# COx2/docker-nvidia-glx-desktop

Hardware: AMD Instinct MI355X
Metric: encoded FPS + p50 end-to-end latency at 1080p60 H.264; concurrent sessions/node (higher is better)
Workload: dtype uint8 video (8-bit 4:2:0), H.264 Constrained Baseline

## Files before the change

### csrc/bindings/module.cpp

```cpp
#include <pybind11/numpy.h>
#include <pybind11/pybind11.h>
#include <pybind11/stl.h>

#include <cstring>

#include "../codec/h264_core.h"
#include "../codec/h264_encoder.h"
#include "../codec/vp8_encoder.h"
#include "../codec/hevc_encoder.h"
#include "../common/hip_check.h"
#include "../common/trace.h"
#include "../kernels/pixel.h"
#include "../runtime/session.h"

namespace py = pybind11;
using namespace mx;

void register_net(py::module& m);
void register_audio(py::module& m);
void register_rfb(py::module& m);

namespace {

template <class T>
T* as_ptr(uintptr_t p) {
    return reinterpret_cast<T*>(p);
}
hipStream_t as_stream(uintptr_t s) { return reinterpret_cast<hipStream_t>(s); }

py::bytes to_bytes(const std::vector<uint8_t>& v) {
    return py::bytes(reinterpret_cast<const char*>(v.data()), v.size());
}

struct PyBits {
    std::vector<uint32_t> words;
    h264::BitWriter w;
    PyBits() : words(4096) { w.init(words.data()); }
    py::tuple finish() {
        const uint32_t bits = w.bits;
        w.flush();
        std::vector<uint8_t> out;
        for (uint32_t i = 0; i < (bits + 7) / 8; ++i) out.push_back((uint8_t)(words[i / 4] >> (24 - 8 * (i % 4))));
        return py::make_tuple(to_bytes(out), bits);
    }
};

py::tuple cavlc_block_py(const std::vector<int>& coef, int nc) {
    PyBits b;
    int16_t c[16] = {0};
    const int n = (int)coef.size();
    if (n != 4 && n != 15 && n != 16) throw std::invalid_argument("block must have 4, 15 or 16 coefficients");
    for (int i = 0; i < n; ++i) c[i] = (int16_t)coef[i];
    h264::cavlc_block(b.w, c, n, nc);
    return b.finish();
}

py::array_t<int> fdct_py(py::array_t<int, py::array::c_style | py::array::forcecast> x) {
    if (x.size() != 16) throw std::invalid_argument("need 16 values");
    py::array_t<int> y(16);
    h264::fdct4x4(x.data(), y.mutable_data());
    return y;
}
py::array_t<int> idct_py(py::array_t<int, py::array::c_style | py::array::forcecast> x) {
    if (x.size() != 16) throw std::invalid_argument("need 16 values");
    py::array_t<int> y(16);
    h264::idct4x4(x.data(), y.mutable_data());
    return y;
}

py::array_t<uint8_t> copy_plane(const uint8_t* dev, int pitch, int w, int h) {
    py::array_t<uint8_t> out({h, w});
    HIP_CHECK(hipDeviceSynchronize());
    HIP_CHECK(hipMemcpy2D(out.mutable_data(), w, dev, pitch, w, h, hipMemcpyDeviceToHost));
    return out;
}

}

PYBIND11_MODULE(_native, m) {
    m.doc() = "mxdesk native runtime: HIP kernels (gfx950), H.264 encoder, session pipeline";

    m.def("device_count", []() {
        int n = 0;
        if (hipGetDeviceCount(&n) != hipSuccess) return 0;
        return n;
    });
    m.def("set_device", [](int d) { HIP_CHECK(hipSetDevice(d)); });
    m.def("device_name", [](int d) {
        hipDeviceProp_t p;
        HIP_CHECK(hipGetDeviceProperties(&p, d));
        return std::string(p.gcnArchName) + " / " + p.name;
    });
    m.def("synchronize", []() { HIP_CHECK(hipDeviceSynchronize()); });
    register_net(m);
    register_audio(m);
    register_rfb(m);
    m.def("now_us", &Session::now_us, "CLOCK_MONOTONIC microseconds (same clock as time.monotonic())");

    py::module h = m.def_submodule("h264", "H.264 building blocks (for tests)");
    h.def("hpel_planes", [](py::array_t<uint8_t, py::array::c_style> ref, int coded_w) {
        if (ref.ndim() != 2 || coded_w % 16 || ref.shape(0) % 16 || ref.shape(1) < coded_w)
            throw std::invalid_argument("ref must be (coded_h, pitch) with 16-aligned coded size");
        int hp = 0;
        auto planes = h264::hpel_planes_for_test(ref.data(), coded_w, (int)ref.shape(0), (int)ref.shape(1), &hp);
        const int rows = (int)ref.shape(0) + 2 * h264::kHpelPad;
        py::list out;
        for (auto& p : planes) {
            py::array_t<uint8_t> a({rows, hp});
            std::memcpy(a.mutable_data(), p.data(), p.size());
            out.append(a);
        }
        return out;
    });
    h.def("mc_luma_gpu", [](py::array_t<uint8_t, py::array::c_style> ref, int coded_w, int x4, int y4) {
        if (ref.ndim() != 2 || coded_w % 16 || ref.shape(0) % 16 || ref.shape(1) < coded_w)
            throw std::invalid_argument("ref must be (coded_h, pitch) with 16-aligned coded size");
        py::array_t<uint8_t> out({16, 16});
        h264::mc_luma_for_test(ref.data(), coded_w, (int)ref.shape(0), (int)ref.shape(1), x4, y4, out.mutable_data());
        return out;
    }, py::arg("ref"), py::arg("coded_w"), py::arg("x4"), py::arg("y4"),
          "16x16 luma prediction at quarter-sample position (x4, y4) by k_inter_encode's interpolation");
    h.def("cavlc_block", &cavlc_block_py, py::arg("coef"), py::arg("nc"));
    h.def("fdct4x4", &fdct_py);
    h.def("idct4x4", &idct_py);
    h.def("ue", [](uint32_t k) {
        PyBits b;
        h264::put_ue(b.w, k);
        return b.finish();
    });
    h.def("se", [](int v) {
        PyBits b;
        h264::put_se(b.w, v);
        return b.finish();
    });
    h.def("luma_qpel", [](py::array_t<uint8_t, py::array::c_style> plane, int x4, int y4) {
        if (plane.ndim() != 2) throw std::invalid_argument("2-D plane");
        const int H = (int)plane.shape(0), W = (int)plane.shape(1);
        return h264::luma_qpel(plane.data(), W, W, H, x4, y4);
    });
    h.def("level_for", &h264::pick_level);
    h.def("zero_sum_4x4", [](int qp) { return h264::zero_sum_4x4(qp); }, py::arg("qp"));
    h.def("zero_sum_chroma_dc", [](int qpc) { return h264::zero_sum_chroma_dc(qpc); }, py::arg("qpc"));
    h.def("chroma_qp", [](int qp, int offset) { return h264::chroma_qp(qp, offset); }, py::arg("qp"),
          py::arg("offset") = 0);
    h.def("quant4x4", [](py::array_t<int, py::array::c_style | py::array::forcecast> y, int qp, bool intra, int start) {
        if (y.size() != 16) throw std::invalid_argument("need 16 values");
        py::array_t<int> z(16);
        const int nz = h264::quant4x4(y.data(), z.mutable_data(), qp, intra, start);
        return py::make_tuple(z, nz);
    }, py::arg("y"), py::arg("qp"), py::arg("intra") = false, py::arg("start") = 0);
    h.def("quant_dc_chroma", [](py::array_t<int, py::array::c_style | py::array::forcecast> dc, int qpc, bool intra) {
        if (dc.size() != 4) throw std::invalid_argument("need 4 values");
        py::array_t<int> z(4);
        const int nz = h264::quant_dc_chroma(dc.data(), z.mutable_data(), qpc, intra);
        return py::make_tuple(z, nz);
    }, py::arg("dc"), py::arg("qpc"), py::arg("intra") = false);
    h.def("luma_block_inter", [](py::array_t<int, py::array::c_style | py::array::forcecast> res, int qp) {
        if (res.size() != 16) throw std::invalid_argument("need 16 values");
        py::array_t<int> z(16), rr(16);
        const int nz = h264::luma_block_inter(res.data(), qp, z.mutable_data(), rr.mutable_data());
        return py::make_tuple(z, rr, nz);
    }, py::arg("res"), py::arg("qp"), "inter luma block: residual (raster) -> levels (scan), reconstructed residual, nz");

    py::class_<h264::EncoderConfig>(m, "EncoderConfig")
        .def(py::init<>())
        .def_readwrite("width", &h264::EncoderConfig::width)
        .def_readwrite("height", &h264::EncoderConfig::height)
        .def_readwrite("fps", &h264::EncoderConfig::fps)
        .def_readwrite("bitrate_kbps", &h264::EncoderConfig::bitrate_kbps)
        .def_readwrite("qp", &h264::EncoderConfig::qp)
        .def_readwrite("qp_min", &h264::EncoderConfig::qp_min)
        .def_readwrite("qp_max", &h264::EncoderConfig::qp_max)
        .def_readwrite("keyint", &h264::EncoderConfig::keyint)
        .def_readwrite("search_range", &h264::EncoderConfig::search_range)
        .def_readwrite("scroll_range", &h264::EncoderConfig::scroll_range)
        .def_readwrite("me_coarse", &h264::EncoderConfig::me_coarse)
        .def_readwrite("intra4x4", &h264::EncoderConfig::intra4x4)
        .def_readwrite("subpel", &h264::EncoderConfig::subpel)
        .def_readwrite("chroma_qp_offset", &h264::EncoderConfig::chroma_qp_offset)
        .def_readwrite("pipeline_depth", &h264::EncoderConfig::pipeline_depth)
        .def_readwrite("aq", &h264::EncoderConfig::aq)
        .def_readwrite("intra_in_p", &h264::EncoderConfig::intra_in_p)
        .def_readwrite("vp8_bpred", &h264::EncoderConfig::vp8_bpred)
        .def_readwrite("vp8_intra", &h264::EncoderConfig::vp8_intra)
        .def_readwrite("mask_x0", &h264::EncoderConfig::mask_x0)
        .def_readwrite("mask_y0", &h264::EncoderConfig::mask_y0)
        .def_readwrite("mask_x1", &h264::EncoderConfig::mask_x1)
        .def_readwrite("mask_y1", &h264::EncoderConfig::mask_y1)
        .def_readwrite("deblock", &h264::EncoderConfig::deblock)
        .def_readwrite("partitions", &h264::EncoderConfig::partitions)
        .def_readwrite("tu_split", &h264::EncoderConfig::tu_split)
        .def_readwrite("hevc_slice_cost", &h264::EncoderConfig::hevc_slice_cost)
        .def_readwrite("hevc_wpp", &h264::EncoderConfig::hevc_wpp)
        .def_readwrite("hevc_wpp_rows", &h264::EncoderConfig::hevc_wpp_rows)
        .def_readwrite("sao", &h264::EncoderConfig::sao)
        .def_readwrite("hevc_chroma_keep", &h264::EncoderConfig::hevc_chroma_keep)
        .def_readwrite("hevc_intra_split", &h264::EncoderConfig::hevc_intra_split);

    py::class_<h264::FrameStats>(m, "FrameStats")
        .def_readonly("frame_index", &h264::FrameStats::frame_index)
        .def_readonly("idr", &h264::FrameStats::idr)
        .def_readonly("qp", &h264::FrameStats::qp)
        .def_readonly("bytes", &h264::FrameStats::bytes)
        .def_readonly("skipped_mbs", &h264::FrameStats::skipped_mbs)
        .def_readonly("encode_ms", &h264::FrameStats::encode_ms)
        .def_property_readonly("sse", [](const h264::FrameStats& s) { return py::make_tuple(s.sse[0], s.sse[1], s.sse[2]); })
        .def_readonly("sse_masked", &h264::FrameStats::sse_masked)
        .def_readonly("masked_pixels", &h264::FrameStats::masked_pixels)
        .def_readonly("deblocked", &h264::FrameStats::deblocked)
        .def_readonly("db_coherent", &h264::FrameStats::db_coherent)
        .def_readonly("db_changed", &h264::FrameStats::db_changed)
        .def_readonly("db_moving", &h264::FrameStats::db_moving)
        .def_readonly("scroll_dx", &h264::FrameStats::scroll_dx)
        .def_readonly("scroll_dy", &h264::FrameStats::scroll_dy);

    py::class_<h264::CpuH264Encoder>(m, "CpuH264Encoder")
        .def(py::init<const h264::EncoderConfig&>())
        .def(
            "encode",
            [](h264::CpuH264Encoder& e, py::array_t<uint8_t, py::array::c_style> y,
               py::array_t<uint8_t, py::array::c_style> uv, bool force_idr) {
                if (y.ndim() != 2 || uv.ndim() != 2 || y.shape(1) != uv.shape(1))
                    throw std::invalid_argument("y (H,P) and uv (H/2,P) planes with equal pitch");
// ... 697 lines not shown
```

### csrc/codec/h264_core.h

```cpp
#pragma once
#include <hip/hip_runtime.h>
#include <stdint.h>

#include "h264_tables.h"

#define MXHD __host__ __device__ __forceinline__

namespace mx {
namespace h264 {

struct BitWriter {
    uint32_t* words;
    uint32_t nwords;
    uint64_t acc;
    int nacc;
    uint32_t bits;

    MXHD void init(uint32_t* w) {
        words = w;
        nwords = 0;
        acc = 0;
        nacc = 0;
        bits = 0;
    }
// ... 455 lines not shown
MXHD Mv predict_mv_skip(MvNb a, MvNb b, MvNb c) {
    if (!a.avail || !b.avail) return Mv{0, 0};
    if (a.ref == 0 && a.mv.x == 0 && a.mv.y == 0) return Mv{0, 0};
    if (b.ref == 0 && b.mv.x == 0 && b.mv.y == 0) return Mv{0, 0};
    return predict_mv16x16(a, b, c);
}

MXHD int cbp_to_codenum(int cbp, bool intra) {
    const uint8_t* t = intra ? kCodeNumToCbpIntra : kCodeNumToCbpInter;
    for (int i = 0; i < 48; ++i)
        if (t[i] == cbp) return i;
    return 0;
}

MXHD int clip255(int v) { return v < 0 ? 0 : (v > 255 ? 255 : v); }

MXHD int ref_px(const uint8_t* p, int pitch, int w, int h, int x, int y) {
    x = x < 0 ? 0 : (x >= w ? w - 1 : x);
    y = y < 0 ? 0 : (y >= h ? h - 1 : y);
    return p[y * pitch + x];
}

MXHD int tap6(int a, int b, int c, int d, int e, int f) { return a - 5 * b + 20 * c + 20 * d - 5 * e + f; }

MXHD int half_h1(const uint8_t* p, int pitch, int w, int h, int x, int y) {
    return tap6(ref_px(p, pitch, w, h, x - 2, y), ref_px(p, pitch, w, h, x - 1, y), ref_px(p, pitch, w, h, x, y),
                ref_px(p, pitch, w, h, x + 1, y), ref_px(p, pitch, w, h, x + 2, y), ref_px(p, pitch, w, h, x + 3, y));
}
MXHD int half_v1(const uint8_t* p, int pitch, int w, int h, int x, int y) {
    return tap6(ref_px(p, pitch, w, h, x, y - 2), ref_px(p, pitch, w, h, x, y - 1), ref_px(p, pitch, w, h, x, y),
                ref_px(p, pitch, w, h, x, y + 1), ref_px(p, pitch, w, h, x, y + 2), ref_px(p, pitch, w, h, x, y + 3));
}

MXHD int luma_qpel(const uint8_t* p, int pitch, int w, int h, int x4, int y4) {
    const int xi = x4 >> 2, yi = y4 >> 2, xf = x4 & 3, yf = y4 & 3;
    const int G = ref_px(p, pitch, w, h, xi, yi);
    if ((xf | yf) == 0) return G;
    auto b_at = [&](int yy) { return clip255((half_h1(p, pitch, w, h, xi, yy) + 16) >> 5); };
    auto h_at = [&](int xx) { return clip255((half_v1(p, pitch, w, h, xx, yi) + 16) >> 5); };
    auto j_val = [&]() {
        int j1 = tap6(half_h1(p, pitch, w, h, xi, yi - 2), half_h1(p, pitch, w, h, xi, yi - 1),
                      half_h1(p, pitch, w, h, xi, yi), half_h1(p, pitch, w, h, xi, yi + 1),
                      half_h1(p, pitch, w, h, xi, yi + 2), half_h1(p, pitch, w, h, xi, yi + 3));
        return clip255((j1 + 512) >> 10);
    };
    if (yf == 0) {
        const int b = b_at(yi);
        if (xf == 2) return b;
        const int other = (xf == 1) ? G : ref_px(p, pitch, w, h, xi + 1, yi);
        return (other + b + 1) >> 1;
    }
    if (xf == 0) {
        const int hh = h_at(xi);
        if (yf == 2) return hh;
        const int other = (yf == 1) ? G : ref_px(p, pitch, w, h, xi, yi + 1);
        return (other + hh + 1) >> 1;
    }
    if (xf == 2 && yf == 2) return j_val();
    if (xf == 2) {
        const int bb = (yf == 1) ? b_at(yi) : b_at(yi + 1);
        return (bb + j_val() + 1) >> 1;
    }
    if (yf == 2) {
        const int hh = (xf == 1) ? h_at(xi) : h_at(xi + 1);
        return (hh + j_val() + 1) >> 1;
    }
    const int bb = (yf == 1) ? b_at(yi) : b_at(yi + 1);
    const int hh = (xf == 1) ? h_at(xi) : h_at(xi + 1);
    return (bb + hh + 1) >> 1;
}

MXHD int chroma_pred8(const uint8_t* uv, int pitch, int cw, int ch, int comp, int x8, int y8) {
    const int xi = x8 >> 3, yi = y8 >> 3, xf = x8 & 7, yf = y8 & 7;
    auto g = [&](int x, int y) {
        x = x < 0 ? 0 : (x >= cw ? cw - 1 : x);
        y = y < 0 ? 0 : (y >= ch ? ch - 1 : y);
        return (int)uv[y * pitch + 2 * x + comp];
    };
    if ((xf | yf) == 0) return g(xi, yi);
    const int A = g(xi, yi), B = g(xi + 1, yi), C = g(xi, yi + 1), D = g(xi + 1, yi + 1);
    return ((8 - xf) * (8 - yf) * A + xf * (8 - yf) * B + (8 - xf) * yf * C + xf * yf * D + 32) >> 6;
}

MXHD int lambda_sad(int qp) {
    constexpr uint8_t tab[52] = {1,  1,  1,  1,  1,  1,  1,  1,  1,  1,  1,  1,  1,  1,  1,  1,  1,  1,
                                 2,  2,  2,  2,  3,  3,  3,  4,  4,  4,  5,  6,  6,  7,  8,  9,  10, 11,
                                 13, 14, 16, 18, 20, 23, 25, 29, 32, 36, 40, 45, 51, 57, 64, 72};
    return tab[qp < 0 ? 0 : (qp > 51 ? 51 : qp)];
}

MXHD int mvd_bits(int d) { return se_len(d); }

}
}
```

### csrc/codec/h264_kernels.hip

```cpp
#include <hip/hip_runtime.h>

#include <cstddef>

#include "../common/hip_check.h"
#include "../common/wave.h"
#include "h264_core.h"
#include "h264_deblock.h"
#include "h264_gpu.h"
#include "h264_mb.h"

namespace mx {
namespace h264 {

namespace {

__device__ __forceinline__ uint32_t bswap32(uint32_t v) { return __builtin_bswap32(v); }

constexpr int kHpTW = 128, kHpTH = 16;
constexpr int kHpSW = kHpTW + 8;
__device__ __forceinline__ int byte_of(uint32_t w, int k) { return (int)((w >> (8 * k)) & 0xff); }
__device__ __forceinline__ uint32_t pack4(int a, int b, int c, int d) {
    const uint32_t lo = __builtin_amdgcn_perm((uint32_t)b, (uint32_t)a, 0x0c0c0400u);
    const uint32_t hi = __builtin_amdgcn_perm((uint32_t)d, (uint32_t)c, 0x0c0c0400u);
    return __builtin_amdgcn_perm(hi, lo, 0x05040100u);
// ... 102 lines not shown
__device__ __forceinline__ int qpel_lds(const uint8_t (*sp)[18][kSpW], int x4, int y4) {
    const int xi = x4 >> 2, yi = y4 >> 2, xf = x4 & 3, yf = y4 & 3;
    const int G = sp[0][yi][xi];
    if ((xf | yf) == 0) return G;
    if (yf == 0) {
        const int b = sp[1][yi][xi];
        if (xf == 2) return b;
        return ((xf == 1 ? G : (int)sp[0][yi][xi + 1]) + b + 1) >> 1;
    }
    if (xf == 0) {
        const int hh = sp[2][yi][xi];
        if (yf == 2) return hh;
        return ((yf == 1 ? G : (int)sp[0][yi + 1][xi]) + hh + 1) >> 1;
    }
    if (xf == 2 && yf == 2) return sp[3][yi][xi];
    if (xf == 2) return ((yf == 1 ? (int)sp[1][yi][xi] : (int)sp[1][yi + 1][xi]) + sp[3][yi][xi] + 1) >> 1;
    if (yf == 2) return ((xf == 1 ? (int)sp[2][yi][xi] : (int)sp[2][yi][xi + 1]) + sp[3][yi][xi] + 1) >> 1;
    const int bb = (yf == 1) ? sp[1][yi][xi] : sp[1][yi + 1][xi];
    const int hh = (xf == 1) ? sp[2][yi][xi] : sp[2][yi][xi + 1];
    return (bb + hh + 1) >> 1;
}

constexpr int kMaxRange = 32;
constexpr int kWinPadX = 4, kWinPadY = 3;
constexpr int kWinStride = 16 + 2 * kMaxRange + 8;
constexpr int kWinRows = 16 + 2 * kMaxRange + 7;
constexpr int kWinWords = kWinRows * kWinStride / 4;

constexpr int kMeThreads = 256, kMeWaves = kMeThreads / 64;
__device__ __forceinline__ uint64_t qsad4(uint32_t hi, uint32_t lo, uint32_t src, uint64_t acc) {
    return __builtin_amdgcn_qsad_pk_u16_u8(((uint64_t)hi << 32) | lo, src, acc);
}
constexpr int kFpRows = 18 + 5;
__device__ __forceinline__ void build_footprints(const uint8_t* win, int org0, int org1, int n,
                                                 uint8_t (*sp)[4][18][kSpW], int16_t (*b1)[kFpRows][kSpW], int tid) {
    for (int i = tid; i < n * kFpRows * 18; i += kMeThreads) {
        const int pi = i / (kFpRows * 18), rem = i - pi * (kFpRows * 18), r = rem / 18, c = rem - r * 18;
        const uint8_t* p = win + (pi ? org1 : org0) + (r - 2) * kWinStride + c;
        b1[pi][r][c] = (int16_t)tap6(p[-2], p[-1], p[0], p[1], p[2], p[3]);
    }
    __syncthreads();
    for (int i = tid; i < n * 324; i += kMeThreads) {
        const int pi = i / 324, rem = i - pi * 324, r = rem / 18, c = rem - r * 18;
        const uint8_t* p = win + (pi ? org1 : org0) + r * kWinStride + c;
        const int16_t(*b)[kSpW] = b1[pi];
        const int v1 = tap6(p[-2 * kWinStride], p[-kWinStride], p[0], p[kWinStride], p[2 * kWinStride], p[3 * kWinStride]);
        const int j1 = tap6(b[r][c], b[r + 1][c], b[r + 2][c], b[r + 3][c], b[r + 4][c], b[r + 5][c]);
        sp[pi][0][r][c] = p[0];
        sp[pi][1][r][c] = (uint8_t)clip255((b[r + 2][c] + 16) >> 5);
        sp[pi][2][r][c] = (uint8_t)clip255((v1 + 16) >> 5);
        sp[pi][3][r][c] = (uint8_t)clip255((j1 + 512) >> 10);
    }
}

struct MeState {
    const uint8_t* ref;
    int qp, search_range, subpel, me_coarse, partitions;
};
__device__ __forceinline__ MeState me_state(const FrameState& f) {
    return MeState{f.me_ref ? f.me_ref : f.ref_y, f.qp, f.search_range, f.subpel, f.me_coarse, f.partitions};
}
__device__ __forceinline__ uint32_t zero_sad_wave(const uint8_t* __restrict__ src_y, const uint8_t* __restrict__ ref,
                                                  int pitch, int x0, int y0, int tid, uint32_t* sw) {
    const int r = tid >> 2, c4 = (tid & 3) * 4;
    *sw = *reinterpret_cast<const uint32_t*>(src_y + (y0 + r) * pitch + x0 + c4);
    const uint32_t rw = *reinterpret_cast<const uint32_t*>(ref + (y0 + r) * pitch + x0 + c4);
    return (uint32_t)wave_sum((int)__builtin_amdgcn_sad_u8(*sw, rw, 0u));
}
__device__ __forceinline__ unsigned long long kmin(unsigned long long a, unsigned long long c) { return c < a ? c : a; }
__device__ __forceinline__ unsigned long long block_min(const unsigned long long* slot) {
    unsigned long long b = slot[0];
    for (int i = 1; i < kMeWaves; ++i) b = kmin(b, slot[i]);
    return b;
}
__device__ __forceinline__ void me_row(const uint32_t* win32, const uint32_t* srcw, int a, int r, uint64_t& lft,
                                       uint64_t& rgt) {
    const uint32_t w0 = win32[a], w1 = win32[a + 1], w2 = win32[a + 2], w3 = win32[a + 3], w4 = win32[a + 4];
    const uint32_t s0 = srcw[r * 4 + 0], s1 = srcw[r * 4 + 1], s2 = srcw[r * 4 + 2], s3 = srcw[r * 4 + 3];
    lft = qsad4(w1, w0, s0, lft);
    lft = qsad4(w2, w1, s1, lft);
    rgt = qsad4(w3, w2, s2, rgt);
    rgt = qsad4(w4, w3, s3, rgt);
}
template <bool kCoarse, class Visit>
__device__ __forceinline__ void me_score16(const uint32_t* win32, const uint32_t* srcw, int ntask, int gw, int side,
                                           int tid, Visit visit) {
    constexpr int kStep = kCoarse ? 2 : 1, kUnroll = kCoarse ? 4 : 2;
    for (int q = tid; q < ntask; q += kMeThreads) {
        const int dyr = kStep * (q / gw), g = q % gw;
        uint64_t acc = 0;
#pragma unroll kUnroll
        for (int r = 0; r < 16; ++r) me_row(win32, srcw, (dyr + r) * (kWinStride / 4) + g, r, acc, acc);
#pragma unroll
        for (int sh = 0; sh < 4; sh += kStep) {
            const int dxr = 4 * g + sh;
            if (dxr >= side) break;
            visit((uint32_t)(acc >> (16 * sh)) & 0xffffu, dxr, dyr);
        }
    }
}
template <int kLanes, class Sad, class Key>
__device__ __forceinline__ unsigned long long me_neighbour(unsigned long long centre, int k, int side, Sad sad,
                                                           Key mkey) {
    const int cb0 = (int)(centre & 0xffff), bxr = cb0 % side, byr = cb0 / side;
    int ddx, ddy;
    subpel_offset(k, &ddx, &ddy);
    const int nxr = bxr + ddx, nyr = byr + ddy;
    const bool inside = nxr >= 0 && nxr < side && nyr >= 0 && nyr < side;
    int d = inside ? sad(nxr, nyr) : 0;
    for (int o = kLanes / 2; o > 0; o >>= 1) d += __shfl_xor(d, o, 64);
    return inside ? mkey((uint32_t)d, nxr, nyr) : ~0ull;
}
template <int kN>
__device__ __forceinline__ void me_refine(const uint8_t (*sp)[4][18][kSpW], uint32_t (*cand)[8], const uint32_t* srcw,
                                          int pi, int k, int sub, int xx, int yy, int lambda, int* vx, int* vy,
                                          uint32_t* cost, bool on = true) {
    const uint32_t s0 = srcw[yy * 4 + (xx >> 2)], s1 = srcw[yy * 4 + (xx >> 2) + 1];
    const int base_x4 = xx * 4 + 4 - vx[pi], base_y4 = yy * 4 + 4 - vy[pi];
    for (int step = 2; step >= 1; step >>= 1) {
        int ddx, ddy;
        subpel_offset(k, &ddx, &ddy);
        const int cx = vx[pi] + ddx * step, cy = vy[pi] + ddy * step;
        int d = 0;
#pragma unroll
        for (int j = 0; j < 8; ++j) {
            d += abs(byte_of(j < 4 ? s0 : s1, j & 3) - qpel_lds(sp[pi], base_x4 + 4 * j + cx, base_y4 + cy));
        }
        if (!on) d = 0;
        for (int o = kMeThreads / (16 * kN); o > 0; o >>= 1) d += __shfl_xor(d, o, 64);
        __syncthreads();
        if (sub == 0) cand[pi][k] = me_cost((uint32_t)d, lambda, cx, cy);
        __syncthreads();
        for (int q = 0; q < kN; ++q) {
            int bdx = 0, bdy = 0;
            uint32_t bcost = cost[q];
            for (int kk = 0; kk < 8; ++kk) {
                const uint32_t cc = cand[q][kk];
                if (cc < bcost) {
                    int ex, ey;
                    subpel_offset(kk, &ex, &ey);
                    bcost = cc;
                    bdx = ex * step;
                    bdy = ey * step;
                }
            }
            vx[q] += bdx;
            vy[q] += bdy;
            cost[q] = bcost;
        }
    }
}
__device__ __forceinline__ MbInfo store_motion(MbInfo* __restrict__ mbs, int mbi, int tid, int cx, int cy, int mvx,
                                               int mvy, int part, const int (&pvx)[2], const int (&pvy)[2]) {
    MbInfo out;
    out.mvx = (int16_t)(4 * cx + mvx);
    out.mvy = (int16_t)(4 * cy + mvy);
    out.part = (uint8_t)part;
    for (int i = 0; i < 2; ++i) {
        out.pmv[2 * i] = part == kPart16x16 ? 0 : (int16_t)(4 * cx + pvx[i]);
        out.pmv[2 * i + 1] = part == kPart16x16 ? 0 : (int16_t)(4 * cy + pvy[i]);
    }
    if (tid == 0) {
        MbInfo& m = mbs[mbi];
        m.mvx = out.mvx;
        m.mvy = out.mvy;
        m.part = out.part;
        for (int i = 0; i < 4; ++i) m.pmv[i] = out.pmv[i];
    }
    return out;
}
__device__ __forceinline__ MbInfo store_motion(MbInfo* __restrict__ mbs, int mbi, int tid, int cx, int cy, int mvx,
                                               int mvy) {
    const int none[2] = {0, 0};
    return store_motion(mbs, mbi, tid, cx, cy, mvx, mvy, kPart16x16, none, none);
}
__device__ __forceinline__ MbInfo store_motion_quads(MbInfo* __restrict__ mbs, int mbi, int tid, int cx, int cy,
                                                     const int (&qvx)[4], const int (&qvy)[4]) {
    MbInfo out;
    out.part = kPart8x8;
#pragma unroll
    for (int q = 0; q < 4; ++q) set_quad_mv(out, q, 4 * cx + qvx[q], 4 * cy + qvy[q]);
    if (tid == 0) {
// ... 25 lines not shown
    const int R = me_range(st.search_range);
    const int W = 16 + 2 * R;
    const uint8_t* __restrict__ ref = st.ref;
    const int lambda = lambda_sad(st.qp);

    constexpr int kWs4 = kWinStride / 4;
    int cx = 0, cy = 0;
    {
        if (tid < 64) {
            uint32_t sw;
            const uint32_t d = zero_sad_wave(src_y, ref, g.pitch, x0, y0, tid, &sw);
            if (tid == 0) s_sad0[0] = d;
        }
        __syncthreads();
        const uint32_t sad0 = s_sad0[0];
        if (sad0 <= static_sad(st.qp)) {
            MbInfo out;
            out.mvx = out.mvy = 0;
            out.part = kPart16x16;
            out.pmv[0] = out.pmv[1] = out.pmv[2] = out.pmv[3] = 0;
            if (tid == 0) {
                MbInfo& m = mbs[mbi];
                m.mvx = 0;
                m.mvy = 0;
                m.part = kPart16x16;
                m.pmv[0] = m.pmv[1] = m.pmv[2] = m.pmv[3] = 0;
            }
            return out;
        }
        if constexpr (kScroll) {
            const int gx = hint[0], gy = hint[1];
            if (gx | gy) {
                if (tid < 64) {
                    const int r = tid >> 2, c4 = (tid & 3) * 4;
                    const uint32_t sw = *reinterpret_cast<const uint32_t*>(src_y + (y0 + r) * g.pitch + x0 + c4);
                    uint32_t rw = 0;
                    for (int k = 0; k < 4; ++k)
                        rw |= (uint32_t)ref_px(ref, g.pitch, g.coded_w, g.coded_h, x0 + gx + c4 + k, y0 + gy + r) << (8 * k);
                    const int d = wave_sum((int)__builtin_amdgcn_sad_u8(sw, rw, 0u));
                    if (tid == 0) s_sad0[1] = (uint32_t)d;
                }
                __syncthreads();
                const int use = scroll_use(s_sad0[1], sad0, st.qp);
                if (use == kScrollExit) return store_motion(mbs, mbi, tid, gx, gy, 0, 0);
                if (use == kScrollCentre) cx = gx, cy = gy;
            }
        }
    }
    const int wrows = W + 2 * kWinPadY + 1, wx0 = x0 + cx - R - kWinPadX, wy0 = y0 + cy - R - kWinPadY;
    const bool dwords = (g.pitch & 3) == 0 && (reinterpret_cast<uintptr_t>(ref) & 3) == 0;
    for (int i = tid; i < wrows * kWs4; i += kMeThreads) {
        const int wy = i / kWs4, wx4 = (i - wy * kWs4) * 4;
        uint32_t w = 0u;
        if (wx4 < W + 2 * kWinPadX) {
            const int py = min(max(wy0 + wy, 0), g.coded_h - 1), px = wx0 + wx4;
            const uint8_t* row = ref + (size_t)py * g.pitch;
            if (kScroll && (wx0 & 3))
                for (int k = 0; k < 4; ++k) w |= (uint32_t)row[min(max(px + k, 0), g.coded_w - 1)] << (8 * k);
            else if (px < 0)
                w = row[0] * 0x01010101u;
            else if (px >= g.coded_w)
                w = row[g.coded_w - 1] * 0x01010101u;
            else if (dwords)
                w = *reinterpret_cast<const uint32_t*>(row + px);
            else
                w = row[px] | ((uint32_t)row[px + 1] << 8) | ((uint32_t)row[px + 2] << 16) | ((uint32_t)row[px + 3] << 24);
        }
        win_lds[i] = w;
    }
    const uint32_t* win32 = win_lds + kWinPadY * kWs4 + kWinPadX / 4;
    auto fp_org = [&](int vx, int vy) {
        return ((vy >> 2) + R + kWinPadY - 1) * kWinStride + (vx >> 2) + R + kWinPadX - 1;
    };
    if (tid < 64) {
        const int r = tid >> 2, c = (tid & 3) * 4;
        srcw[tid] = *reinterpret_cast<const uint32_t*>(src_y + (y0 + r) * g.pitch + x0 + c);
    }
    __syncthreads();

    const int side = 2 * R + 1, gw = (side + 3) >> 2, ngroups = side * gw;
    unsigned long long best = ~0ull;
    const bool coarse = st.me_coarse != 0;
    const bool parts = st.partitions != 0;
    auto mkey = [&](uint32_t sad, int dxr, int dyr) {
        const int dx = dxr - R, dy = dyr - R;
        const uint32_t cost = me_cost(sad, lambda, 4 * dx, 4 * dy);
        const uint32_t dist = (uint32_t)(abs(dx) + abs(dy));
        return ((unsigned long long)cost << 32) | (dist << 16) | (uint32_t)(dyr * side + dxr);
    };
    unsigned long long pb[4] = {~0ull, ~0ull, ~0ull, ~0ull};
    unsigned long long qb[4] = {~0ull, ~0ull, ~0ull, ~0ull};
    auto visit_quads = [&](const uint32_t* qd, int dxr, int dyr) {
        if constexpr (kQuad)
            for (int i = 0; i < 4; ++i) qb[i] = kmin(qb[i], mkey(qd[i], dxr, dyr));
        best = kmin(best, mkey(qd[0] + qd[1] + qd[2] + qd[3], dxr, dyr));
        pb[0] = kmin(pb[0], mkey(qd[0] + qd[1], dxr, dyr));
        pb[1] = kmin(pb[1], mkey(qd[2] + qd[3], dxr, dyr));
        pb[2] = kmin(pb[2], mkey(qd[0] + qd[2], dxr, dyr));
        pb[3] = kmin(pb[3], mkey(qd[1] + qd[3], dxr, dyr));
    };
    if (parts) {
        const int nsh = coarse ? 2 : 4, ntp = coarse ? (R + 1) * gw : ngroups;
        for (int q = tid; q < ntp; q += kMeThreads) {
            const int dyr = coarse ? 2 * (q / gw) : q / gw, g = q % gw;
            uint64_t acc[4] = {0, 0, 0, 0};
#pragma unroll
            for (int h = 0; h < 2; ++h)
#pragma unroll 2
                for (int r = 8 * h; r < 8 * h + 8; ++r)
                    me_row(win32, srcw, (dyr + r) * kWs4 + g, r, acc[2 * h], acc[2 * h + 1]);
#pragma unroll
            for (int si = 0; si < 4; ++si) {
                if (si >= nsh) break;
                const int dxr = 4 * g + (coarse ? 2 * si : si);
                if (dxr >= side) break;
                const int sh = 16 * (coarse ? 2 * si : si);
                const uint32_t qd[4] = {(uint32_t)(acc[0] >> sh) & 0xffffu, (uint32_t)(acc[1] >> sh) & 0xffffu,
                                        (uint32_t)(acc[2] >> sh) & 0xffffu, (uint32_t)(acc[3] >> sh) & 0xffffu};
                visit_quads(qd, dxr, dyr);
            }
        }
    } else {
        auto visit = [&](uint32_t sad, int dxr, int dyr) { best = kmin(best, mkey(sad, dxr, dyr)); };
        if (coarse)
            me_score16<true>(win32, srcw, (R + 1) * gw, gw, side, tid, visit);
        else
            me_score16<false>(win32, srcw, ngroups, gw, side, tid, visit);
    }
    best = wave_min_u64(best);
    if (lane == 0) red[tid >> 6] = best;
    __shared__ unsigned long long pred4[4][kMeWaves];
    if (parts) {
#pragma unroll
        for (int sh = 0; sh < 4; ++sh) {
            const unsigned long long v = wave_min_u64(pb[sh]);
            if (lane == 0) pred4[sh][tid >> 6] = v;
        }
    }
    __shared__ unsigned long long qred4[kQuad ? 4 : 1][kMeWaves];
    if constexpr (kQuad) {
        if (parts) {
#pragma unroll
            for (int i = 0; i < 4; ++i) {
                const unsigned long long v = wave_min_u64(qb[i]);
                if (lane == 0) qred4[i][tid >> 6] = v;
            }
        }
    }
    __syncthreads();
    unsigned long long b = block_min(red);
    unsigned long long pbest[4] = {~0ull, ~0ull, ~0ull, ~0ull};
    if (parts)
        for (int sh = 0; sh < 4; ++sh) pbest[sh] = block_min(pred4[sh]);
    unsigned long long qbest[4] = {~0ull, ~0ull, ~0ull, ~0ull};
    if constexpr (kQuad) {
        if (parts)
            for (int i = 0; i < 4; ++i) qbest[i] = block_min(qred4[i]);
    }
    const uint8_t* wb = reinterpret_cast<const uint8_t*>(win32);
    const uint8_t* sb = reinterpret_cast<const uint8_t*>(srcw);
    if (parts && coarse) {
        __shared__ unsigned long long pnkey[4][8];
        const int ev = tid >> 3, sub = tid & 7, sh = ev >> 3, k = ev & 7;
        const unsigned long long nk = me_neighbour<8>(pbest[sh], k, side, [&](int nxr, int nyr) {
            int d = 0;
            for (int part_row = 0; part_row < 2; ++part_row) {
                const int rr = sh < 2 ? (sh == 0 ? sub : 8 + sub) : 2 * sub + part_row;
                const int c0 = sh < 2 ? 8 * part_row : (sh == 2 ? 0 : 8);
#pragma unroll
                for (int j = 0; j < 8; ++j)
                    d += abs((int)sb[rr * 16 + c0 + j] - (int)wb[(nyr + rr) * kWinStride + nxr + c0 + j]);
            }
            return d;
        }, mkey);
        if (sub == 0) pnkey[sh][k] = nk;
        __syncthreads();
        for (int s2 = 0; s2 < 4; ++s2)
            for (int i = 0; i < 8; ++i) pbest[s2] = kmin(pbest[s2], pnkey[s2][i]);
        if constexpr (kQuad) {
            __shared__ unsigned long long qnkey[4][8];
            const int qi = ev >> 3;
            const unsigned long long qk = me_neighbour<8>(qbest[qi], k, side, [&](int nxr, int nyr) {
                const int rr = 8 * (qi >> 1) + sub, c0 = 8 * (qi & 1);
                int d = 0;
#pragma unroll
                for (int j = 0; j < 8; ++j)
                    d += abs((int)sb[rr * 16 + c0 + j] - (int)wb[(nyr + rr) * kWinStride + nxr + c0 + j]);
                return d;
            }, mkey);
            if (sub == 0) qnkey[qi][k] = qk;
            __syncthreads();
            for (int s2 = 0; s2 < 4; ++s2)
                for (int i = 0; i < 8; ++i) qbest[s2] = kmin(qbest[s2], qnkey[s2][i]);
        }
    }
    if (coarse) {
        __shared__ unsigned long long nkey[8];
        const int k = tid >> 5, sub = tid & 31, py = sub >> 1, px0 = (sub & 1) * 8;
        const unsigned long long nk = me_neighbour<32>(b, k, side, [&](int nxr, int nyr) {
            const uint8_t* wrow = wb + (nyr + py) * kWinStride + nxr + px0;
            const uint32_t s0 = srcw[py * 4 + (px0 >> 2)], s1 = srcw[py * 4 + (px0 >> 2) + 1];
            int d = 0;
#pragma unroll
            for (int j = 0; j < 8; ++j) d += abs(byte_of(j < 4 ? s0 : s1, j & 3) - (int)wrow[j]);
            return d;
        }, mkey);
        if (sub == 0) nkey[k] = nk;
        __syncthreads();
        for (int i = 0; i < 8; ++i) b = kmin(b, nkey[i]);
    }
// ... 2307 lines not shown
```

### csrc/codec/h264_mb.h

```cpp
#pragma once
#include "h264_core.h"
#include "h264_gpu.h"
#include "h264_intra.h"

namespace mx {
namespace h264 {

constexpr int kNumRoles = 28;

struct Avail {
    bool left, top, topright, topleft;
};

MXHD Avail mb_avail(const Geometry& g, int mbx, int mby, int slice_rows) {
    Avail a;
    const bool top_same_slice = mby > 0 && (mby / slice_rows) == ((mby - 1) / slice_rows);
    a.left = mbx > 0;
    a.top = top_same_slice;
    a.topright = top_same_slice && mbx < g.mb_w - 1;
    a.topleft = top_same_slice && mbx > 0;
    return a;
}

MXHD int combine_nc(bool ha, int na, bool hb, int nb) {
// ... 312 lines not shown
            const Mv v = quad_mv(m, q);
            bits += mvd_bits(v.x) + mvd_bits(v.y);
        }
        return satd + (uint32_t)(lambda_sad(frame_qp) * bits);
    }
    return satd + (uint32_t)(lambda_sad(frame_qp) *
                             (mvd_bits(m.pmv[0]) + mvd_bits(m.pmv[1]) + mvd_bits(m.pmv[2]) + mvd_bits(m.pmv[3])));
}

MXHD int idr_slice_rows(int mb_h) {
    const int ns = (mb_h + 3) / 4;
    return (mb_h + ns - 1) / ns;
}

MXHD int qp_delta(int qp, int pred) { return ((qp - pred + 26 + 52) % 52) - 26; }

MXHD SliceParams make_slice_params(int first_mb, int idr, int frame_num, int log2_max_frame_num, int idr_pic_id,
                                   int qp_delta, int deblock_off) {
    SliceParams sp;
    sp.first_mb = first_mb;
    sp.idr = idr;
    sp.frame_num = frame_num;
    sp.log2_max_frame_num = log2_max_frame_num;
    sp.idr_pic_id = idr_pic_id;
    sp.qp_delta = qp_delta;
    sp.disable_deblock = deblock_off;
    return sp;
}


MXHD int luma_block_inter(const int* res, int qp, int* zscan, int* rres) {
    int y[16], z[16], d[16];
    fdct4x4(res, y);
    const int nz = quant4x4(y, z, qp, false, 0);
    for (int k = 0; k < 16; ++k) zscan[k] = z[kZigzag4x4[k]];
    dequant4x4(z, d, qp, 0);
    idct4x4(d, rres);
    return nz;
}

constexpr int fdct_row_gain(int i) { return (i & 1) ? 2 : 1; }
constexpr int zero_sum_4x4_calc(int qp) {
    const int qm = qp % 6, qbits = 15 + qp / 6;
    const int room = (1 << qbits) - 1 - (1 << qbits) / 6;
    int t = room;
    for (int i = 0; i < 16; ++i) {
        const int b = room / (fdct_row_gain(i >> 2) * fdct_row_gain(i & 3) * kQuantMF[qm][kPosClass[i]]);
        t = b < t ? b : t;
    }
    return t;
}
constexpr int zero_sum_chroma_dc_calc(int qpc) {
    const int qm = qpc % 6, qbits = 16 + qpc / 6;
    const int room = (1 << qbits) - 1 - 2 * ((1 << (qbits - 1)) / 6);
    return room / kQuantMF[qm][0];
}
struct ZeroSumTab {
    uint16_t blk[52], cdc[52];
    constexpr ZeroSumTab() : blk{}, cdc{} {
        for (int q = 0; q < 52; ++q) {
            const int a = zero_sum_4x4_calc(q), b = zero_sum_chroma_dc_calc(q);
            blk[q] = (uint16_t)(a > 0xffff ? 0xffff : a);
            cdc[q] = (uint16_t)(b > 0xffff ? 0xffff : b);
        }
    }
};
MXHD int zero_sum_4x4(int qp) {
    constexpr ZeroSumTab tab;
    return tab.blk[qp < 0 ? 0 : (qp > 51 ? 51 : qp)];
}
MXHD int zero_sum_chroma_dc(int qpc) {
    constexpr ZeroSumTab tab;
    return tab.cdc[qpc < 0 ? 0 : (qpc > 51 ? 51 : qpc)];
}

MXHD uint32_t me_cost(uint32_t sad, int lambda, int mvx, int mvy) {
    return sad + (uint32_t)(lambda * (mvd_bits(mvx) + mvd_bits(mvy)));
}

MXHD int me_range(int r) {
    r = r < 4 ? 4 : (r > 32 ? 32 : r);
    return (r + 3) & ~3;
}
constexpr uint32_t kStaticSad = 128;
MXHD uint32_t static_sad(int qp) {
    const uint32_t t = 64u * (uint32_t)lambda_sad(qp);
    return t > kStaticSad ? t : kStaticSad;
}

constexpr int kScrollMaxReach = 192;
MXHD int scroll_reach(int r) {
    r = r < 0 ? 0 : (r > kScrollMaxReach ? kScrollMaxReach : r);
    return (r + 3) & ~3;
}
constexpr int kScrollLattice = 2;
MXHD bool scroll_is_probe(int mbx, int mby) { return mbx % kScrollLattice == 0 && mby % kScrollLattice == 0; }
MXHD int scroll_probes_x(int mb_w) { return (mb_w + kScrollLattice - 1) / kScrollLattice; }
MXHD int scroll_probes_y(int mb_h) { return (mb_h + kScrollLattice - 1) / kScrollLattice; }
constexpr uint32_t kScrollMinVotes = 3;
MXHD int scroll_bins(int D) { return 2 * (2 * D + 1); }
MXHD int scroll_bin(int axis, int d, int D) { return axis * (2 * D + 1) + d + D; }
MXHD unsigned long long scroll_probe_key(uint32_t sad, int axis, int d, int D) {
    const uint32_t ad = (uint32_t)(d < 0 ? -d : d);
    return ((unsigned long long)sad << 32) | (ad << 16) | (uint32_t)scroll_bin(axis, d, D);
}
MXHD bool scroll_key_votes(unsigned long long k, int qp) { return (uint32_t)(k >> 32) <= static_sad(qp); }
MXHD int scroll_key_bin(unsigned long long k) { return (int)(k & 0xffffu); }
MXHD unsigned long long scroll_bin_key(uint32_t votes, int bin, int D) {
    if (!votes) return 0ull;
    const int axis = bin / (2 * D + 1), d = bin % (2 * D + 1) - D;
    const uint32_t ad = (uint32_t)(d < 0 ? -d : d);
    return ((unsigned long long)votes << 32) | ((0xfffu - ad) << 16) | ((uint32_t)(1 - axis) << 15) |
           ((uint32_t)(d < 0) << 14) | (uint32_t)bin;
}
MXHD void scroll_decide(unsigned long long best, uint32_t total, int D, int* gx, int* gy) {
    const uint32_t votes = (uint32_t)(best >> 32);
    *gx = *gy = 0;
    if (votes < kScrollMinVotes || 2u * votes < total) return;
    const int bin = (int)(best & 0x3fffu), axis = bin / (2 * D + 1), d = bin % (2 * D + 1) - D;
    if (axis) *gx = d; else *gy = d;
}
static_assert(2 * (2 * kScrollMaxReach + 1) < (1 << 14), "scroll_bin_key keeps the bin in 14 bits");
enum ScrollUse : int { kScrollExit = 0, kScrollCentre = 1, kScrollZero = 2 };
MXHD int scroll_use(uint32_t sadg, uint32_t sad0, int qp) {
    return sadg <= static_sad(qp) ? kScrollExit : (sadg < sad0 ? kScrollCentre : kScrollZero);
}

MXHD void subpel_offset(int k, int* dx, int* dy) {
    *dx = (k < 3) ? (k - 1) : (k == 3 ? -1 : (k == 4 ? 1 : (k - 6)));
    *dy = (k < 3) ? -1 : ((k == 3 || k == 4) ? 0 : 1);
}

}
}
```

Before: 13250.

## Pack motion-search candidate keys into 32 bits and widen once per thread

The full-search motion estimation kernel now compares candidates with a 32-bit key: cost, distance, and a small per-thread visit number packed together. The MV-bit cost per axis is precomputed with a clz formula, and the winner is decoded back to the 64-bit key only once per thread before the wave reduction. This replaces 64-bit key building and compares (cost, abs, multiply) in the hot inner loop with cheap 32-bit adds and mins, including for partition and quad minima. Static asserts bound the field widths and Python bindings check ordering equivalence, but correctness depends on the packing matching the task map exactly.

```diff
diff --git a/csrc/bindings/module.cpp b/csrc/bindings/module.cpp
--- a/csrc/bindings/module.cpp
+++ b/csrc/bindings/module.cpp
@@ -44,6 +44,46 @@
         return py::make_tuple(to_bytes(out), bits);
     }
 };
+
+py::tuple me_key_check_py(int R, int lambda, bool coarse, const std::vector<uint32_t>& sads) {
+    using namespace h264;
+    if (R != me_range(R)) throw std::invalid_argument("R must be a search range me_range() returns");
+    const int side = 2 * R + 1, gw = me_group_width(R), ntask = me_tasks(R, coarse), step = coarse ? 2 : 1;
+    const uint32_t nmask = (1u << kMeKeyNumBits) - 1;
+    long long bad = 0, pairs = 0;
+    int most = 0;
+    struct Cand { uint32_t term; int dxr, dyr; };
+    for (int tid = 0; tid < kMeSearchThreads; ++tid) {
+        std::vector<Cand> v;
+        uint32_t n0 = 0;
+        for (int q = tid; q < ntask; q += kMeSearchThreads, n0 += 4) {
+            const int dyr = step * (q / gw), g = q % gw;
+            const uint32_t ty = me_key_axis(lambda, dyr - R) + n0;
+            for (int sh = 0; sh < 4; sh += step) {
+                const int dxr = 4 * g + sh;
+                if (dxr >= side) break;
+                v.push_back({ty + me_key_axis(lambda, dxr - R) + (uint32_t)sh, dxr, dyr});
+            }
+        }
+        most = std::max(most, (int)v.size());
+        if (v.empty() && me_key_widen(~0u, tid, R, coarse) != ~0ull) ++bad;
+        for (size_t i = 0; i < v.size(); ++i) {
+            if (i && v[i].dyr * side + v[i].dxr <= v[i - 1].dyr * side + v[i - 1].dxr) ++bad;
+            if (i && (v[i].term & nmask) <= (v[i - 1].term & nmask)) ++bad;
+            for (size_t j = i; j < v.size(); ++j)
+                for (uint32_t sa : sads)
+                    for (uint32_t sb : sads) {
+                        const uint32_t na = me_key32(sa, v[i].term), nb = me_key32(sb, v[j].term);
+                        const unsigned long long wa = me_key64(sa, lambda, R, v[i].dxr, v[i].dyr),
+                                                 wb = me_key64(sb, lambda, R, v[j].dxr, v[j].dyr);
+                        ++pairs;
+                        if ((na < nb) != (wa < wb) || (na == nb) != (wa == wb)) ++bad;
+                        if (me_key_widen(std::min(na, nb), tid, R, coarse) != std::min(wa, wb)) ++bad;
+                    }
+        }
+    }
+    return py::make_tuple(bad, pairs, most);
+}
 
 py::tuple cavlc_block_py(const std::vector<int>& coef, int nc) {
     PyBits b;
@@ -139,6 +179,24 @@
         return h264::luma_qpel(plane.data(), W, W, H, x4, y4);
     });
     h.def("level_for", &h264::pick_level);
+    h.def("me_range", [](int r) { return h264::me_range(r); });
+    h.def("lambda_sad", [](int qp) { return h264::lambda_sad(qp); });
+    h.def("mvd_bits", [](int d) { return h264::mvd_bits(d); });
+    h.def("me_mvd_bits4", [](int d) { return h264::me_mvd_bits4(d); });
+    h.def("me_tasks", [](int R, bool coarse) { return h264::me_tasks(R, coarse); }, py::arg("R"), py::arg("coarse"));
+    h.def("me_key64", [](uint32_t sad, int lambda, int R, int dxr, int dyr) {
+        return h264::me_key64(sad, lambda, R, dxr, dyr);
+    }, py::arg("sad"), py::arg("lambda_"), py::arg("R"), py::arg("dxr"), py::arg("dyr"));
+    h.def("me_key_axis", [](int lambda, int d) { return h264::me_key_axis(lambda, d); });
+    h.def("me_key32", [](uint32_t sad, uint32_t term) { return h264::me_key32(sad, term); });
+    h.def("me_key_widen", [](uint32_t key, int tid, int R, bool coarse) {
+        return h264::me_key_widen(key, tid, R, coarse);
+    }, py::arg("key"), py::arg("tid"), py::arg("R"), py::arg("coarse"));
+    h.def("me_key_check", &me_key_check_py, py::arg("R"), py::arg("lambda_"), py::arg("coarse"), py::arg("sads"));
+    h.attr("ME_MAX_RANGE") = h264::kMeMaxRange;
+    h.attr("ME_SEARCH_THREADS") = h264::kMeSearchThreads;
+    h.attr("ME_MAX_LAMBDA") = h264::kMeMaxLambda;
+    h.attr("ME_KEY_BITS") = py::make_tuple(h264::kMeKeyNumBits, h264::kMeKeyDistBits, h264::kMeKeyCostBits);
     h.def("zero_sum_4x4", [](int qp) { return h264::zero_sum_4x4(qp); }, py::arg("qp"));
     h.def("zero_sum_chroma_dc", [](int qpc) { return h264::zero_sum_chroma_dc(qpc); }, py::arg("qpc"));
     h.def("chroma_qp", [](int qp, int offset) { return h264::chroma_qp(qp, offset); }, py::arg("qp"),
diff --git a/csrc/codec/h264_core.h b/csrc/codec/h264_core.h
--- a/csrc/codec/h264_core.h
+++ b/csrc/codec/h264_core.h
@@ -561,7 +561,7 @@
     return ((8 - xf) * (8 - yf) * A + xf * (8 - yf) * B + (8 - xf) * yf * C + xf * yf * D + 32) >> 6;
 }
 
-MXHD int lambda_sad(int qp) {
+MXHD constexpr int lambda_sad(int qp) {
     constexpr uint8_t tab[52] = {1,  1,  1,  1,  1,  1,  1,  1,  1,  1,  1,  1,  1,  1,  1,  1,  1,  1,
                                  2,  2,  2,  2,  3,  3,  3,  4,  4,  4,  5,  6,  6,  7,  8,  9,  10, 11,
                                  13, 14, 16, 18, 20, 23, 25, 29, 32, 36, 40, 45, 51, 57, 64, 72};
diff --git a/csrc/codec/h264_kernels.hip b/csrc/codec/h264_kernels.hip
--- a/csrc/codec/h264_kernels.hip
+++ b/csrc/codec/h264_kernels.hip
@@ -208,22 +208,28 @@
     rgt = qsad4(w3, w2, s2, rgt);
     rgt = qsad4(w4, w3, s3, rgt);
 }
-template <bool kCoarse, class Visit>
-__device__ __forceinline__ void me_score16(const uint32_t* win32, const uint32_t* srcw, int ntask, int gw, int side,
-                                           int tid, Visit visit) {
+static_assert(kMaxRange == kMeMaxRange && kMeThreads == kMeSearchThreads, "me_key_widen's task map");
+template <bool kCoarse>
+__device__ __forceinline__ uint32_t me_score16(const uint32_t* win32, const uint32_t* srcw, int ntask, int gw, int side,
+                                               int tid, int R, int lambda) {
     constexpr int kStep = kCoarse ? 2 : 1, kUnroll = kCoarse ? 4 : 2;
-    for (int q = tid; q < ntask; q += kMeThreads) {
+    uint32_t best = ~0u;
+    uint32_t n0 = 0;
+    for (int q = tid; q < ntask; q += kMeThreads, n0 += 4) {
         const int dyr = kStep * (q / gw), g = q % gw;
         uint64_t acc = 0;
 #pragma unroll kUnroll
         for (int r = 0; r < 16; ++r) me_row(win32, srcw, (dyr + r) * (kWinStride / 4) + g, r, acc, acc);
+        const uint32_t ty = me_key_axis(lambda, dyr - R) + n0;
 #pragma unroll
         for (int sh = 0; sh < 4; sh += kStep) {
             const int dxr = 4 * g + sh;
             if (dxr >= side) break;
-            visit((uint32_t)(acc >> (16 * sh)) & 0xffffu, dxr, dyr);
-        }
-    }
+            const uint32_t term = ty + me_key_axis(lambda, dxr - R) + (uint32_t)sh;
+            best = min(best, me_key32((uint32_t)(acc >> (16 * sh)) & 0xffffu, term));
+        }
+    }
+    return best;
 }
 template <int kLanes, class Sad, class Key>
 __device__ __forceinline__ unsigned long long me_neighbour(unsigned long long centre, int k, int side, Sad sad,
@@ -415,26 +421,23 @@
     unsigned long long best = ~0ull;
     const bool coarse = st.me_coarse != 0;
     const bool parts = st.partitions != 0;
-    auto mkey = [&](uint32_t sad, int dxr, int dyr) {
-        const int dx = dxr - R, dy = dyr - R;
-        const uint32_t cost = me_cost(sad, lambda, 4 * dx, 4 * dy);
-        const uint32_t dist = (uint32_t)(abs(dx) + abs(dy));
-        return ((unsigned long long)cost << 32) | (dist << 16) | (uint32_t)(dyr * side + dxr);
-    };
+    auto mkey = [&](uint32_t sad, int dxr, int dyr) { return me_key64(sad, lambda, R, dxr, dyr); };
     unsigned long long pb[4] = {~0ull, ~0ull, ~0ull, ~0ull};
     unsigned long long qb[4] = {~0ull, ~0ull, ~0ull, ~0ull};
-    auto visit_quads = [&](const uint32_t* qd, int dxr, int dyr) {
-        if constexpr (kQuad)
-            for (int i = 0; i < 4; ++i) qb[i] = kmin(qb[i], mkey(qd[i], dxr, dyr));
-        best = kmin(best, mkey(qd[0] + qd[1] + qd[2] + qd[3], dxr, dyr));
-        pb[0] = kmin(pb[0], mkey(qd[0] + qd[1], dxr, dyr));
-        pb[1] = kmin(pb[1], mkey(qd[2] + qd[3], dxr, dyr));
-        pb[2] = kmin(pb[2], mkey(qd[0] + qd[2], dxr, dyr));
-        pb[3] = kmin(pb[3], mkey(qd[1] + qd[3], dxr, dyr));
-    };
     if (parts) {
-        const int nsh = coarse ? 2 : 4, ntp = coarse ? (R + 1) * gw : ngroups;
-        for (int q = tid; q < ntp; q += kMeThreads) {
+        uint32_t nbest = ~0u, npb[4] = {~0u, ~0u, ~0u, ~0u}, nqb[4] = {~0u, ~0u, ~0u, ~0u};
+        auto visit_quads = [&](const uint32_t* qd, uint32_t term) {
+            if constexpr (kQuad)
+                for (int i = 0; i < 4; ++i) nqb[i] = min(nqb[i], me_key32(qd[i], term));
+            nbest = min(nbest, me_key32(qd[0] + qd[1] + qd[2] + qd[3], term));
+            npb[0] = min(npb[0], me_key32(qd[0] + qd[1], term));
+            npb[1] = min(npb[1], me_key32(qd[2] + qd[3], term));
+            npb[2] = min(npb[2], me_key32(qd[0] + qd[2], term));
+            npb[3] = min(npb[3], me_key32(qd[1] + qd[3], term));
+        };
+        const int ntp = coarse ? (R + 1) * gw : ngroups;
+        uint32_t n0 = 0;
+        for (int q = tid; q < ntp; q += kMeThreads, n0 += 4) {
             const int dyr = coarse ? 2 * (q / gw) : q / gw, g = q % gw;
             uint64_t acc[4] = {0, 0, 0, 0};
 #pragma unroll
@@ -442,23 +445,29 @@
 #pragma unroll 2
                 for (int r = 8 * h; r < 8 * h + 8; ++r)
                     me_row(win32, srcw, (dyr + r) * kWs4 + g, r, acc[2 * h], acc[2 * h + 1]);
-#pragma unroll
-            for (int si = 0; si < 4; ++si) {
-                if (si >= nsh) break;
-                const int dxr = 4 * g + (coarse ? 2 * si : si);
+            const uint32_t ty = me_key_axis(lambda, dyr - R) + n0;
+#pragma unroll
+            for (int wsh = 0; wsh < 4; ++wsh) {
+                if (coarse && (wsh & 1)) continue;
+                const int dxr = 4 * g + wsh;
                 if (dxr >= side) break;
-                const int sh = 16 * (coarse ? 2 * si : si);
+                const int sh = 16 * wsh;
                 const uint32_t qd[4] = {(uint32_t)(acc[0] >> sh) & 0xffffu, (uint32_t)(acc[1] >> sh) & 0xffffu,
                                         (uint32_t)(acc[2] >> sh) & 0xffffu, (uint32_t)(acc[3] >> sh) & 0xffffu};
-                visit_quads(qd, dxr, dyr);
-            }
+                visit_quads(qd, ty + me_key_axis(lambda, dxr - R) + (uint32_t)wsh);
+            }
+        }
+        best = me_key_widen(nbest, tid, R, coarse);
+#pragma unroll
+        for (int i = 0; i < 4; ++i) pb[i] = me_key_widen(npb[i], tid, R, coarse);
+        if constexpr (kQuad) {
+#pragma unroll
+            for (int i = 0; i < 4; ++i) qb[i] = me_key_widen(nqb[i], tid, R, coarse);
         }
     } else {
-        auto visit = [&](uint32_t sad, int dxr, int dyr) { best = kmin(best, mkey(sad, dxr, dyr)); };
-        if (coarse)
-            me_score16<true>(win32, srcw, (R + 1) * gw, gw, side, tid, visit);
-        else
-            me_score16<false>(win32, srcw, ngroups, gw, side, tid, visit);
+        const uint32_t nbest = coarse ? me_score16<true>(win32, srcw, (R + 1) * gw, gw, side, tid, R, lambda)
+                                      : me_score16<false>(win32, srcw, ngroups, gw, side, tid, R, lambda);
+        best = me_key_widen(nbest, tid, R, coarse);
     }
     best = wave_min_u64(best);
     if (lane == 0) red[tid >> 6] = best;
diff --git a/csrc/codec/h264_mb.h b/csrc/codec/h264_mb.h
--- a/csrc/codec/h264_mb.h
+++ b/csrc/codec/h264_mb.h
@@ -418,6 +418,49 @@
     r = r < 4 ? 4 : (r > 32 ? 32 : r);
     return (r + 3) & ~3;
 }
+constexpr int kMeMaxRange = 32;
+constexpr int kMeSearchThreads = 256;
+MXHD unsigned long long me_key64(uint32_t sad, int lambda, int R, int dxr, int dyr) {
+    const int dx = dxr - R, dy = dyr - R;
+    const uint32_t cost = me_cost(sad, lambda, 4 * dx, 4 * dy);
+    const uint32_t dist = (uint32_t)((dx < 0 ? -dx : dx) + (dy < 0 ? -dy : dy));
+    return ((unsigned long long)cost << 32) | (dist << 16) | (uint32_t)(dyr * (2 * R + 1) + dxr);
+}
+MXHD constexpr int me_group_width(int R) { return (2 * R + 1 + 3) >> 2; }
+MXHD constexpr int me_tasks(int R, bool coarse) { return (coarse ? R + 1 : 2 * R + 1) * me_group_width(R); }
+constexpr int kMeKeyNumBits = 5, kMeKeyDistBits = 7, kMeKeyCostShift = kMeKeyNumBits + kMeKeyDistBits;
+constexpr int kMeMaxLambda = 72;
+MXHD constexpr uint32_t me_mvd_bits4(int d) {
+    const uint32_t ad = (uint32_t)(d < 0 ? -d : d);
+    return 63u - 2u * (uint32_t)__builtin_clz(8u * ad + (d <= 0 ? 1u : 0u));
+}
+static_assert(4 * ((me_tasks(kMeMaxRange, false) + kMeSearchThreads - 1) / kMeSearchThreads) <= (1 << kMeKeyNumBits) &&
+                  4 * ((me_tasks(kMeMaxRange, true) + kMeSearchThreads - 1) / kMeSearchThreads) <= (1 << kMeKeyNumBits),
+              "a thread's visit numbers fit the key's low field");
+static_assert(2 * kMeMaxRange < (1 << kMeKeyDistBits), "|dx| + |dy| fits the key's distance field");
+static_assert(me_mvd_bits4(kMeMaxRange) == 17 && me_mvd_bits4(-kMeMaxRange) == 17 && me_mvd_bits4(0) == 1 &&
+                  me_mvd_bits4(1) == 7 && me_mvd_bits4(-1) == 7,
+              "se(4 d) lengths");
+constexpr int kMeKeyCostBits = 17;
+static_assert(lambda_sad(51) == kMeMaxLambda && lambda_sad(0) == 1, "lambda_sad() grows with qp up to kMeMaxLambda");
+static_assert(256u * 255u + (uint32_t)kMeMaxLambda * 2u * me_mvd_bits4(kMeMaxRange) < (1u << kMeKeyCostBits),
+              "the cost fits kMeKeyCostBits");
+static_assert(kMeKeyCostBits + kMeKeyCostShift < 32, "a key stays below 2^31: ~0 is no candidate's key");
+MXHD uint32_t me_key_axis(int lambda, int d) {
+    const uint32_t ad = (uint32_t)(d < 0 ? -d : d);
+    return (((uint32_t)lambda * me_mvd_bits4(d)) << kMeKeyCostShift) + (ad << kMeKeyNumBits);
+}
+MXHD uint32_t me_key32(uint32_t sad, uint32_t term) { return (sad << kMeKeyCostShift) + term; }
+MXHD unsigned long long me_key_widen(uint32_t key, int tid, int R, bool coarse) {
+    if (key == ~0u) return ~0ull;
+    const int n = (int)(key & ((1u << kMeKeyNumBits) - 1)), q = tid + kMeSearchThreads * (n >> 2), gw = me_group_width(R);
+    static_assert((kMeSearchThreads << (kMeKeyNumBits - 2)) * me_group_width(kMeMaxRange) <= (1 << 16), "q gw < 2^16");
+    const int row = (int)(((uint32_t)q * (uint32_t)(((1 << 16) + gw - 1) / gw)) >> 16);
+    const int dyr = (coarse ? 2 : 1) * row, dxr = 4 * (q - row * gw) + (n & 3);
+    const uint32_t dist = (key >> kMeKeyNumBits) & ((1u << kMeKeyDistBits) - 1);
+    return ((unsigned long long)(key >> kMeKeyCostShift) << 32) | (dist << 16) | (uint32_t)(dyr * (2 * R + 1) + dxr);
+}
+
 constexpr uint32_t kStaticSad = 128;
 MXHD uint32_t static_sad(int qp) {
     const uint32_t t = 64u * (uint32_t)lambda_sad(qp);
```

After: 13240. About the same (-0.1%).
